# lturing/ORB_SLAM3_modified

Measured on AMD Instinct MI355X. Metric: ORB features/ms (+ frames/s), 640x480 8-level pyramid, 1000 features/frame, higher is better.
Workload: dtype u8

## Files before the change

### orb_slam3_modified_amd/csrc/orbx_kernels.hip

```cpp
#include <hip/hip_runtime.h>

#include "glibc_sincosf.h"
#include "gnu_sort.h"
#include "orbx_internal.h"

namespace orbx {

__constant__ __align__(16) int8_t c_pattern[1024] = {
#include "orb_pattern.inc"
};

__device__ __forceinline__ int fast_div(int n, uint32_t M) { return M ? (int)__umulhi((uint32_t)n, M) : n; }

__device__ __forceinline__ int mul_i24(int a, int b) {
  int r;
  asm("v_mul_i32_i24 %0, %1, %2" : "=v"(r) : "v"(a), "v"(b));
  return r;
}

__device__ __forceinline__ uint32_t mul_u24(uint32_t a, uint32_t b) {
  uint32_t r;
  asm("v_mul_u32_u24 %0, %1, %2" : "=v"(r) : "v"(a), "v"(b));
  return r;
}

__device__ __forceinline__ int xcd_logical_block(int n_items) {
  const int chunk = (int)(gridDim.x >> 3);
// ... 185 lines not shown
      *(uint32_t*)(B + r * bp + 4 * c) = v;
    }
  }
  __syncthreads();
#pragma unroll
  for (int k = 1; k <= K; k++) {
    const ChainLevel& L = a.lv[k - 1];
    const uint8_t* prev = smem + a.buf_off[k - 1];
    const int pp = a.buf_pitch[k - 1];
    const int nd = (X1[k] - X0[k] + 4) >> 2, nr = Y1[k] - Y0[k] + 1;
    uint8_t* outp = L.dst + (long long)frame * a.dst_frame_stride;
    const uint32_t m = nd > 1 ? (uint32_t)(((1ull << 32) + nd - 1) / nd) : 0u;
    for (int i = t; i < nd * nr; i += T) {
      const int r = fast_div(i, m), c = i - r * nd;
      const int y = Y0[k] + r, x4 = X0[k] + 4 * c;
      const uint32_t packed = chain_px4(prev, pp, X0[k - 1], Y0[k - 1], L.xt, L.yt[y], x4, L.w);
      if (x4 < ((L.w + 3) & ~3)) *(uint32_t*)(outp + (long long)y * L.pitch + x4) = packed;
      if (k < K) *(uint32_t*)(smem + a.buf_off[k] + r * a.buf_pitch[k] + 4 * c) = packed;
    }
    if (k < K) __syncthreads();
  }
}

__device__ __forceinline__ uint32_t umin3(uint32_t a, uint32_t b, uint32_t c) { return min(min(a, b), c); }
__device__ __forceinline__ uint32_t umax3(uint32_t a, uint32_t b, uint32_t c) { return max(max(a, b), c); }

__device__ __forceinline__ int fast_score16(int v, const uint32_t (&p)[16]) {
  uint32_t M3[16], m3[16];
#pragma unroll
  for (int k = 0; k < 16; k++) {
    M3[k] = umax3(p[k], p[(k + 1) & 15], p[(k + 2) & 15]);
    m3[k] = umin3(p[k], p[(k + 1) & 15], p[(k + 2) & 15]);
  }
  uint32_t M9[16], m9[16];
#pragma unroll
  for (int k = 0; k < 16; k++) {
    M9[k] = umax3(M3[k], M3[(k + 3) & 15], M3[(k + 6) & 15]);
    m9[k] = umin3(m3[k], m3[(k + 3) & 15], m3[(k + 6) & 15]);
  }
  uint32_t minmax = umin3(M9[0], M9[1], M9[2]), maxmin = umax3(m9[0], m9[1], m9[2]);
#pragma unroll
  for (int k = 3; k < 15; k += 2) {
    minmax = umin3(minmax, M9[k], M9[k + 1]);
    maxmin = umax3(maxmin, m9[k], m9[k + 1]);
  }
  minmax = min(minmax, M9[15]);
  maxmin = max(maxmin, m9[15]);
  return max(v - (int)minmax, (int)maxmin - v) - 1;
}

typedef unsigned short u16x2_t __attribute__((ext_vector_type(2)));
__device__ __forceinline__ u16x2_t as_u16x2(uint32_t x) { u16x2_t r; __builtin_memcpy(&r, &x, 4); return r; }
__device__ __forceinline__ uint32_t as_u32(u16x2_t x) { uint32_t r; __builtin_memcpy(&r, &x, 4); return r; }

__device__ __forceinline__ uint32_t fast_pretest_pk(uint32_t c, uint32_t p0, uint32_t p8, uint32_t p4, uint32_t p12, uint32_t p2,
                                                    uint32_t p10, uint32_t p6, uint32_t p14, uint32_t t_hi) {
  const u16x2_t a0 = as_u16x2(p0), a8 = as_u16x2(p8), a4 = as_u16x2(p4), a12 = as_u16x2(p12);
  const u16x2_t a2 = as_u16x2(p2), a10 = as_u16x2(p10), a6 = as_u16x2(p6), a14 = as_u16x2(p14);
  const u16x2_t maxmin = __builtin_elementwise_max(
      __builtin_elementwise_max(__builtin_elementwise_min(a0, a8), __builtin_elementwise_min(a4, a12)),
      __builtin_elementwise_max(__builtin_elementwise_min(a2, a10), __builtin_elementwise_min(a6, a14)));
  const u16x2_t minmax = __builtin_elementwise_min(
      __builtin_elementwise_min(__builtin_elementwise_max(a0, a8), __builtin_elementwise_max(a4, a12)),
      __builtin_elementwise_min(__builtin_elementwise_max(a2, a10), __builtin_elementwise_max(a6, a14)));
  const u16x2_t T = as_u16x2(t_hi);
  const u16x2_t lo = __builtin_elementwise_sub_sat(as_u16x2(c & 0xff00ff00u), T);
  const u16x2_t hi = __builtin_elementwise_add_sat(as_u16x2(c | 0x00ff00ffu), T);
  return as_u32(__builtin_elementwise_sub_sat(lo, maxmin)) | as_u32(__builtin_elementwise_sub_sat(minmax, hi));
}

__device__ __forceinline__ uint32_t fast_pretest_pk_lo(uint32_t c, uint32_t p0, uint32_t p8, uint32_t p4, uint32_t p12, uint32_t p2,
                                                       uint32_t p10, uint32_t p6, uint32_t p14, uint32_t t_lo) {
  const u16x2_t a0 = as_u16x2(p0), a8 = as_u16x2(p8), a4 = as_u16x2(p4), a12 = as_u16x2(p12);
  const u16x2_t a2 = as_u16x2(p2), a10 = as_u16x2(p10), a6 = as_u16x2(p6), a14 = as_u16x2(p14);
  const u16x2_t maxmin = __builtin_elementwise_max(
      __builtin_elementwise_max(__builtin_elementwise_min(a0, a8), __builtin_elementwise_min(a4, a12)),
// ... 124 lines not shown
        ps[j] = (dark | bright) & valid & (act != 0);
      }
      const unsigned long long b0 = __ballot(ps[0]), b1 = __ballot(ps[1]), b2 = __ballot(ps[2]), b3 = __ballot(ps[3]);
      const int n0 = __popcll(b0), n1_ = __popcll(b1), n2 = __popcll(b2), n3 = __popcll(b3);
      const int tot = n0 + n1_ + n2 + n3;
      if (tot) {
        int base = 0;
        if (lane == 0) base = atomicAdd(&s_cnt, tot);
        base = __builtin_amdgcn_readfirstlane(base);
        const int ent = c0 + (ry << 7);
        const int o0 = __builtin_amdgcn_mbcnt_hi((uint32_t)(b0 >> 32), __builtin_amdgcn_mbcnt_lo((uint32_t)b0, base));
        const int o1 = __builtin_amdgcn_mbcnt_hi((uint32_t)(b1 >> 32), __builtin_amdgcn_mbcnt_lo((uint32_t)b1, base + n0));
        const int o2 = __builtin_amdgcn_mbcnt_hi((uint32_t)(b2 >> 32), __builtin_amdgcn_mbcnt_lo((uint32_t)b2, base + n0 + n1_));
        const int o3 = __builtin_amdgcn_mbcnt_hi((uint32_t)(b3 >> 32), __builtin_amdgcn_mbcnt_lo((uint32_t)b3, base + n0 + n1_ + n2));
        if (ps[0]) list[o0] = (uint16_t)ent;
        if (ps[1]) list[o1] = (uint16_t)(ent + 1);
        if (ps[2]) list[o2] = (uint16_t)(ent + 2);
        if (ps[3]) list[o3] = (uint16_t)(ent + 3);
      }
    }
  }
  __syncthreads();
  n1 = s_cnt;
  for (int e = t; e < n1; e += T) {
    const int ent = list[e];
    const int x = ent & 127, y = ent >> 7;
    const uint8_t* c0 = tile + y * PITCH + (x + xo);
    const int v = c0[3 * PITCH + 3];
    uint32_t p[16];
    p[0] = c0[6 * PITCH + 3];  p[1] = c0[6 * PITCH + 4];  p[2] = c0[5 * PITCH + 5];  p[3] = c0[4 * PITCH + 6];
    p[4] = c0[3 * PITCH + 6];  p[5] = c0[2 * PITCH + 6];  p[6] = c0[1 * PITCH + 5];  p[7] = c0[4];
    p[8] = c0[3];              p[9] = c0[2];              p[10] = c0[1 * PITCH + 1]; p[11] = c0[2 * PITCH];
    p[12] = c0[3 * PITCH];     p[13] = c0[4 * PITCH];     p[14] = c0[5 * PITCH + 1]; p[15] = c0[6 * PITCH + 2];
    const int s = fast_score16(v, p);
    if (s >= TH && s > 0) sc[(y + 1) * PITCH + (x + 1)] = (uint8_t)s;
  }
  __syncthreads();
  int any_ini = 0;
  for (int e = t; e < n1; e += T) {
    const int ent = list[e];
    const int x = ent & 127, y = ent >> 7;
    const uint8_t* q = sc + y * PITCH + x;
    const int s = q[PITCH + 1];
    if (s > 0) {
      const int m = max(max(max((int)q[0], (int)q[1]), max((int)q[2], (int)q[PITCH])),
                        max(max((int)q[PITCH + 2], (int)q[2 * PITCH]), max((int)q[2 * PITCH + 1], (int)q[2 * PITCH + 2])));
      if (s > m) {
        list[e] = (uint16_t)(ent | 0x8000);
        any_ini |= twopass ? 1 : (int)(s >= ini_th);
      }
    }
  }
  const int use_ini = __syncthreads_or(any_ini);
  if (!twopass) { TH = use_ini ? ini_th : min_th; break; }
  if (use_ini || pass == 1 || ini_th == min_th) break;
  TH = min_th;
  if (t == 0) s_cnt = 0;
  __syncthreads();
// ... 1887 lines not shown
    if constexpr (LDSP) {
      const uint8_t* sp = s_patch[w * K + k];
      const int lctr = 18 * kDescSlicePitch + 18 + ((kx - 18) & 3);
      if (brief_fma) brief_taps<true, kDescSlicePitch>(sp, lctr, kDescSlicePitch, pat, a, b, t0, t1);
      else brief_taps<false, kDescSlicePitch>(sp, lctr, kDescSlicePitch, pat, a, b, t0, t1);
    } else {
      if (brief_fma) brief_taps<true, 0>(bplane, ctr, bp, pat, a, b, t0, t1);
      else brief_taps<false, 0>(bplane, ctr, bp, pat, a, b, t0, t1);
    }
    const unsigned long long b0 = __ballot(t0[0] < t1[0]), b1 = __ballot(t0[1] < t1[1]), b2 = __ballot(t0[2] < t1[2]), b3 = __ballot(t0[3] < t1[3]);
    uint32_t word = 0;
    asm("s_nop 4\n\tv_writelane_b32 %0, %1, 0\n\tv_writelane_b32 %0, %2, 1\n\tv_writelane_b32 %0, %3, 2\n\tv_writelane_b32 %0, %4, 3\n\t"
        "v_writelane_b32 %0, %5, 4\n\tv_writelane_b32 %0, %6, 5\n\tv_writelane_b32 %0, %7, 6\n\tv_writelane_b32 %0, %8, 7"
        : "+v"(word)
        : "s"((uint32_t)b0), "s"((uint32_t)(b0 >> 32)), "s"((uint32_t)b1), "s"((uint32_t)(b1 >> 32)), "s"((uint32_t)b2), "s"((uint32_t)(b2 >> 32)),
          "s"((uint32_t)b3), "s"((uint32_t)(b3 >> 32)));
    if (lane < 8) *(uint32_t*)(out_desc + ((long long)frame * g->out_cap + slot) * 32 + lane * 4) = word;
    if (mirror_desc && lane < 8) *(uint32_t*)(mirror_desc + ((long long)frame * g->out_cap + slot) * 32 + lane * 4) = word;
  }
}

constexpr int kFB_ROWS = 43, kFB_PITCH = 48, kFB_X0 = 24, kFB_Y0 = 21, kFB_HP_ROWS = 22, kFB_HP_COLS = 40, kFB_BPITCH = 40;
#include "fb_items.inc"

template <int K, int R>
__global__ __launch_bounds__(256) void k_describe_blur(const DeviceGeom* __restrict__ g, const uint8_t* __restrict__ imgs,
                                                       long long img_row_stride, long long img_frame_stride,
                                                       const uint8_t* __restrict__ pyr, long long pyr_frame_bytes,
                                                       const uint2* __restrict__ kp_list, const int32_t* __restrict__ counts,
                                                       orbx_keypoint* __restrict__ out_kps, uint8_t* __restrict__ out_desc,
                                                       BlurConsts bc, int groups_per_frame, int nitems, uint32_t m_gpf,
                                                       int atan_fma, int brief_fma) {
  const int lane = threadIdx.x & 63, w = __builtin_amdgcn_readfirstlane(threadIdx.x >> 6);
  const int L = xcd_logical_block(nitems);
  if (L < 0) return;
  const int frame = fast_div(L, m_gpf);
  const int total = counts[frame * 2];
  const int first = (L - frame * groups_per_frame) * R * 4 * K;
  if (first >= total) return;
  char4 pat[4];
#pragma unroll
  for (int q = 0; q < 4; q++) pat[q] = ((const char4*)c_pattern)[q * 64 + lane];
  int wu[4], wv[4];
  {
    const uint4 a = ((const uint4*)c_fb_w)[2 * lane], b = ((const uint4*)c_fb_w)[2 * lane + 1];
    wu[0] = (int)a.x; wu[1] = (int)a.y; wu[2] = (int)a.z; wu[3] = (int)a.w;
    wv[0] = (int)b.x; wv[1] = (int)b.y; wv[2] = (int)b.z; wv[3] = (int)b.w;
  }
  __shared__ __align__(16) uint8_t s_raw[4 * K][kFB_ROWS * kFB_PITCH + 16];
  __shared__ __align__(16) uint32_t s_hp[4][kFB_HP_ROWS * kFB_HP_COLS];
  int h_r0[3], h_r1[3], h_hp[3], v_hp[3], v_b[3];
  {
    uint32_t o[16];
#pragma unroll
    for (int i = 0; i < 4; i++) {
      const uint4 q = ((const uint4*)c_fb_off)[4 * lane + i];
      o[4 * i] = q.x; o[4 * i + 1] = q.y; o[4 * i + 2] = q.z; o[4 * i + 3] = q.w;
    }
#pragma unroll
    for (int t = 0; t < 3; t++) { h_r0[t] = (int)o[5 * t]; h_r1[t] = (int)o[5 * t + 1]; h_hp[t] = (int)o[5 * t + 2]; v_hp[t] = (int)o[5 * t + 3]; v_b[t] = (int)o[5 * t + 4]; }
  }
  __shared__ int s_mom[4 * K][2];
  __shared__ float s_trig[4 * K][3];
  uint32_t* hp = s_hp[w];
#pragma unroll 1
  for (int rnd = 0; rnd < R; rnd++) {
  const int gfirst = first + rnd * 4 * K;
  if (gfirst >= total) break;
  const int g0 = gfirst + w * K;
  const int nk = max(0, min(K, total - g0));
  uint2 rec = make_uint2(0u, 0u);
  if (lane < nk) rec = kp_list[(long long)frame * g->out_cap + g0 + lane];
  if (rnd) __syncthreads();
  int my_m01 = 0, my_m10 = 0;
  __builtin_amdgcn_sched_barrier(0);
  if (nk > 0) {
    bool fast[K];
#pragma unroll
    for (int k = 0; k < K; k++) {
      const int kk = min(k, nk - 1);
      const uint32_t p = __builtin_amdgcn_readlane(rec.x, kk);
      const int l = (int)(__builtin_amdgcn_readlane(rec.y, kk) & 0xffu);
      const DeviceLevel& lv = g->lv[l];
// ... 66 lines not shown
      const uint32_t dwv[4] = {a.x, a.y, b.x, b.y};
      int m10 = 0, m01 = 0;
#pragma unroll
      for (int i = 0; i < 4; i++) {
        const int px = (int)(dwv[i] ^ 0x80808080u);
        m10 = __builtin_amdgcn_sdot4(px, wu[i], m10, false);
        m01 = __builtin_amdgcn_sdot4(px, wv[i], m01, false);
      }
      m10 = __builtin_amdgcn_readlane(wave_sum_lane63(m10), 63);
      m01 = __builtin_amdgcn_readlane(wave_sum_lane63(m01), 63);
      if (lane == k) { my_m10 = m10; my_m01 = m01; }
    }
  }
  if (lane < nk) { s_mom[w * K + lane][0] = my_m01; s_mom[w * K + lane][1] = my_m10; }
  __syncthreads();
  if (w == 0 && lane < 4 * K) {
    const float ang = fast_atan2_deg((float)s_mom[lane][0], (float)s_mom[lane][1], atan_fma);
    const float factorPI = (float)(3.14159265358979323846 / 180.f);
    const float rad = __fmul_rn(ang, factorPI);
    s_trig[lane][0] = ang; s_trig[lane][1] = orbx_glibc::cosf_exact(rad); s_trig[lane][2] = orbx_glibc::sinf_exact(rad);
  }
  __syncthreads();
  float my_a = 0.f, my_b = 0.f;
  if (lane < nk) {
    my_a = s_trig[w * K + lane][1]; my_b = s_trig[w * K + lane][2];
    const int l = (int)(rec.y & 0xffu), slot = (int)(rec.y >> 8);
    const DeviceLevel& lv = g->lv[l];
    orbx_keypoint kp;
    float fx = (float)pt_x(rec.x), fy = (float)pt_y(rec.x);
    if (l != 0) { fx = __fmul_rn(fx, lv.scale); fy = __fmul_rn(fy, lv.scale); }
    kp.x = fx; kp.y = fy; kp.size = (float)lv.scaled_patch; kp.angle = s_trig[w * K + lane][0]; kp.response = (float)pt_s(rec.x);
    kp.octave = l; kp.class_id = -1;
    out_kps[(long long)frame * g->out_cap + slot] = kp;
  }
#pragma unroll 1
  for (int k = 0; k < nk; k++) {
    const int slot = (int)(__builtin_amdgcn_readlane(rec.y, k) >> 8);
    const float a = __uint_as_float(__builtin_amdgcn_readlane(__float_as_uint(my_a), k));
    const float b = __uint_as_float(__builtin_amdgcn_readlane(__float_as_uint(my_b), k));
    uint8_t* sp = s_raw[w * K + k];
#pragma unroll
    for (int t = 0; t < 3; t++) {
      uint32_t ha[4], hb[4];
      hrow4((const uint32_t*)(sp + h_r0[t]), bc, ha);
      hrow4((const uint32_t*)(sp + h_r1[t]), bc, hb);
      uint4 o;
      o.x = __builtin_amdgcn_perm(hb[0], ha[0], 0x05040100u); o.y = __builtin_amdgcn_perm(hb[1], ha[1], 0x05040100u);
      o.z = __builtin_amdgcn_perm(hb[2], ha[2], 0x05040100u); o.w = __builtin_amdgcn_perm(hb[3], ha[3], 0x05040100u);
      if (t < 2 || lane + 128 < kFB_NH) *(uint4*)((uint8_t*)hp + h_hp[t]) = o;
    }
    wave_lds_sync();
#pragma unroll
    for (int t = 0; t < 3; t++) {
      uint4 P[4];
#pragma unroll
      for (int q = 0; q < 4; q++) P[q] = *(const uint4*)((const uint8_t*)hp + v_hp[t] + q * (kFB_HP_COLS * 4));
      uint32_t e[4], o[4];
#pragma unroll
      for (int c = 0; c < 4; c++) {
        const uint32_t p0 = c == 0 ? P[0].x : c == 1 ? P[0].y : c == 2 ? P[0].z : P[0].w;
        const uint32_t p1 = c == 0 ? P[1].x : c == 1 ? P[1].y : c == 2 ? P[1].z : P[1].w;
        const uint32_t p2 = c == 0 ? P[2].x : c == 1 ? P[2].y : c == 2 ? P[2].z : P[2].w;
        const uint32_t p3 = c == 0 ? P[3].x : c == 1 ? P[3].y : c == 2 ? P[3].z : P[3].w;
        e[c] = udot2(p3, bc.we[3], udot2(p2, bc.we[2], udot2(p1, bc.we[1], udot2(p0, bc.we[0], bc.radd))));
        o[c] = udot2(p3, bc.wo[3], udot2(p2, bc.wo[2], udot2(p1, bc.wo[1], udot2(p0, bc.wo[0], bc.radd))));
      }
      const uint32_t pe = __builtin_amdgcn_perm(__builtin_amdgcn_perm(e[3], e[2], 0x0c0c0602u), __builtin_amdgcn_perm(e[1], e[0], 0x0c0c0602u), 0x05040100u);
      const uint32_t po = __builtin_amdgcn_perm(__builtin_amdgcn_perm(o[3], o[2], 0x0c0c0602u), __builtin_amdgcn_perm(o[1], o[0], 0x0c0c0602u), 0x05040100u);
      if (t < 2 || lane + 128 < kFB_NV) {
        *(uint32_t*)(sp + v_b[t]) = pe;
        *(uint32_t*)(sp + v_b[t] + kFB_BPITCH) = po;
      }
    }
    wave_lds_sync();
    int t0[4], t1[4];
    const int lctr = 18 * kFB_BPITCH + 20;
    char4 patk[4];
#pragma unroll
    for (int q = 0; q < 4; q++) {
      uint32_t pq;
      __builtin_memcpy(&pq, &pat[q], 4);
      asm volatile("" : "+v"(pq));
      __builtin_memcpy(&patk[q], &pq, 4);
    }
    if (brief_fma) brief_taps<true, kFB_BPITCH>(sp, lctr, kFB_BPITCH, patk, a, b, t0, t1);
    else brief_taps<false, kFB_BPITCH>(sp, lctr, kFB_BPITCH, patk, a, b, t0, t1);
    const unsigned long long b0 = __ballot(t0[0] < t1[0]), b1 = __ballot(t0[1] < t1[1]), b2 = __ballot(t0[2] < t1[2]), b3 = __ballot(t0[3] < t1[3]);
    uint32_t word = 0;
    asm("s_nop 4\n\tv_writelane_b32 %0, %1, 0\n\tv_writelane_b32 %0, %2, 1\n\tv_writelane_b32 %0, %3, 2\n\tv_writelane_b32 %0, %4, 3\n\t"
        "v_writelane_b32 %0, %5, 4\n\tv_writelane_b32 %0, %6, 5\n\tv_writelane_b32 %0, %7, 6\n\tv_writelane_b32 %0, %8, 7"
        : "+v"(word)
        : "s"((uint32_t)b0), "s"((uint32_t)(b0 >> 32)), "s"((uint32_t)b1), "s"((uint32_t)(b1 >> 32)), "s"((uint32_t)b2), "s"((uint32_t)(b2 >> 32)),
          "s"((uint32_t)b3), "s"((uint32_t)(b3 >> 32)));
    if (lane < 8) *(uint32_t*)(out_desc + ((long long)frame * g->out_cap + slot) * 32 + lane * 4) = word;
  }
// ... 109 lines not shown
```

Before: 331,700.

## Pack FAST scoring two-per-lane and bin vertical blur work by keypoint angle

FAST corner scoring now handles two candidates per thread. Pixel values are packed into f16x2 lanes and reinterpreted as f16 bit patterns, so packed min/max extrema can halve the scoring ALU work. The descriptor blur's vertical pass now reads per-lane offsets from precomputed angle-binned tables (16 orientation bins). Only the blurred pixels that the rotated BRIEF pattern can touch are computed, cutting three passes to two. The cost is a large constant table, per-keypoint bin lookup, and reliance on small-integer f16 bit patterns ordering correctly under min/max.

```diff
diff --git a/orb_slam3_modified_amd/csrc/fb_vbins.inc b/orb_slam3_modified_amd/csrc/fb_vbins.inc
--- /dev/null
+++ b/orb_slam3_modified_amd/csrc/fb_vbins.inc
@@ -0,0 +1,260 @@
+constexpr int kFB_VBINS = 16;
+constexpr int kFB_NV_BIN[kFB_VBINS] = {123, 120, 119, 118, 118, 119, 118, 116, 116, 120, 120, 121, 121, 120, 121, 124};
+__constant__ __align__(16) uint32_t c_fb_vbin_off[kFB_VBINS * 64 * 4] = {
+  48, 12, 1488, 732, 192, 88, 1504, 736, 208, 92, 1520, 740, 224, 96, 1536, 744,
+  336, 164, 1552, 748, 352, 168, 1568, 752, 368, 172, 1616, 804, 384, 176, 1632, 808,
+  400, 180, 1648, 812, 416, 184, 1664, 816, 432, 188, 1680, 820, 448, 192, 1696, 824,
+  496, 244, 1712, 828, 512, 248, 1728, 832, 528, 252, 1776, 884, 544, 256, 1792, 888,
+  560, 260, 1808, 892, 576, 264, 1824, 896, 592, 268, 1840, 900, 608, 272, 1856, 904,
+  656, 324, 1872, 908, 672, 328, 1888, 912, 688, 332, 1920, 960, 704, 336, 1936, 964,
+  720, 340, 1952, 968, 736, 344, 1968, 972, 752, 348, 1984, 976, 768, 352, 2000, 980,
+  784, 356, 2016, 984, 816, 404, 2032, 988, 832, 408, 2048, 992, 848, 412, 2096, 1044,
+  864, 416, 2112, 1048, 880, 420, 2128, 1052, 896, 424, 2144, 1056, 912, 428, 2160, 1060,
+  928, 432, 2176, 1064, 944, 436, 2192, 1068, 976, 484, 2208, 1072, 992, 488, 2256, 1124,
+  1008, 492, 2272, 1128, 1024, 496, 2288, 1132, 1040, 500, 2304, 1136, 1056, 504, 2320, 1140,
+  1072, 508, 2336, 1144, 1088, 512, 2352, 1148, 1136, 564, 2368, 1152, 1152, 568, 2416, 1204,
+  1168, 572, 2432, 1208, 1184, 576, 2448, 1212, 1200, 580, 2464, 1216, 1216, 584, 2480, 1220,
+  1232, 588, 2496, 1224, 1248, 592, 2512, 1228, 1296, 644, 2528, 1232, 1312, 648, 2640, 1300,
+  1328, 652, 2656, 1304, 1344, 656, 2672, 1308, 1360, 660, 2816, 1384, 1376, 664, 2816, 1384,
+  1392, 668, 2816, 1384, 1408, 672, 2816, 1384, 1456, 724, 2816, 1384, 1472, 728, 2816, 1384,
+  48, 12, 1488, 732, 64, 16, 1504, 736, 80, 20, 1520, 740, 208, 92, 1536, 744,
+  224, 96, 1552, 748, 240, 100, 1568, 752, 256, 104, 1584, 756, 352, 168, 1600, 800,
+  368, 172, 1616, 804, 384, 176, 1632, 808, 400, 180, 1648, 812, 416, 184, 1664, 816,
+  512, 248, 1680, 820, 528, 252, 1696, 824, 544, 256, 1712, 828, 560, 260, 1728, 832,
+  576, 264, 1760, 880, 592, 268, 1776, 884, 672, 328, 1792, 888, 688, 332, 1808, 892,
+  704, 336, 1824, 896, 720, 340, 1840, 900, 736, 344, 1856, 904, 752, 348, 1872, 908,
+  768, 352, 1888, 912, 832, 408, 1920, 960, 848, 412, 1936, 964, 864, 416, 1952, 968,
+  880, 420, 1968, 972, 896, 424, 1984, 976, 912, 428, 2000, 980, 928, 432, 2016, 984,
+  944, 436, 2032, 988, 976, 484, 2096, 1044, 992, 488, 2112, 1048, 1008, 492, 2128, 1052,
+  1024, 496, 2144, 1056, 1040, 500, 2160, 1060, 1056, 504, 2176, 1064, 1072, 508, 2192, 1068,
+  1088, 512, 2288, 1132, 1104, 516, 2304, 1136, 1136, 564, 2320, 1140, 1152, 568, 2336, 1144,
+  1168, 572, 2352, 1148, 1184, 576, 2448, 1212, 1200, 580, 2464, 1216, 1216, 584, 2480, 1220,
+  1232, 588, 2496, 1224, 1248, 592, 2512, 1228, 1264, 596, 2624, 1296, 1280, 640, 2640, 1300,
+  1296, 644, 2656, 1304, 1312, 648, 2784, 1376, 1328, 652, 2800, 1380, 1344, 656, 2816, 1384,
+  1360, 660, 2816, 1384, 1376, 664, 2816, 1384, 1392, 668, 2816, 1384, 1408, 672, 2816, 1384,
+  1424, 676, 2816, 1384, 1440, 720, 2816, 1384, 1456, 724, 2816, 1384, 1472, 728, 2816, 1384,
+  64, 16, 1504, 736, 80, 20, 1520, 740, 96, 24, 1536, 744, 224, 96, 1552, 748,
+  240, 100, 1568, 752, 256, 104, 1584, 756, 272, 108, 1616, 804, 368, 172, 1632, 808,
+  384, 176, 1648, 812, 400, 180, 1664, 816, 416, 184, 1680, 820, 432, 188, 1696, 824,
+  528, 252, 1712, 828, 544, 256, 1728, 832, 560, 260, 1744, 836, 576, 264, 1776, 884,
+  592, 268, 1792, 888, 656, 324, 1808, 892, 672, 328, 1824, 896, 688, 332, 1840, 900,
+  704, 336, 1856, 904, 720, 340, 1872, 908, 736, 344, 1888, 912, 752, 348, 1904, 916,
+  816, 404, 1952, 968, 832, 408, 1968, 972, 848, 412, 1984, 976, 864, 416, 2000, 980,
+  880, 420, 2016, 984, 896, 424, 2032, 988, 912, 428, 2048, 992, 960, 480, 2064, 996,
+  976, 484, 2112, 1048, 992, 488, 2128, 1052, 1008, 492, 2144, 1056, 1024, 496, 2160, 1060,
+  1040, 500, 2176, 1064, 1056, 504, 2192, 1068, 1072, 508, 2208, 1072, 1088, 512, 2272, 1128,
+  1120, 560, 2288, 1132, 1136, 564, 2304, 1136, 1152, 568, 2320, 1140, 1168, 572, 2336, 1144,
+  1184, 576, 2352, 1148, 1200, 580, 2448, 1212, 1216, 584, 2464, 1216, 1232, 588, 2480, 1220,
+  1248, 592, 2496, 1224, 1264, 596, 2608, 1292, 1280, 640, 2624, 1296, 1296, 644, 2640, 1300,
+  1312, 648, 2768, 1372, 1328, 652, 2784, 1376, 1344, 656, 2800, 1380, 1360, 660, 2800, 1380,
+  1376, 664, 2800, 1380, 1392, 668, 2800, 1380, 1408, 672, 2800, 1380, 1424, 676, 2800, 1380,
+  1440, 720, 2800, 1380, 1456, 724, 2800, 1380, 1472, 728, 2800, 1380, 1488, 732, 2800, 1380,
+  96, 24, 1504, 736, 112, 28, 1520, 740, 240, 100, 1536, 744, 256, 104, 1552, 748,
+  272, 108, 1568, 752, 336, 164, 1632, 808, 352, 168, 1648, 812, 368, 172, 1664, 816,
+  384, 176, 1680, 820, 400, 180, 1696, 824, 416, 184, 1712, 828, 432, 188, 1728, 832,
+  448, 192, 1792, 888, 496, 244, 1808, 892, 512, 248, 1824, 896, 528, 252, 1840, 900,
+  544, 256, 1856, 904, 560, 260, 1872, 908, 576, 264, 1888, 912, 592, 268, 1904, 916,
+  608, 272, 1952, 968, 656, 324, 1968, 972, 672, 328, 1984, 976, 688, 332, 2000, 980,
+  704, 336, 2016, 984, 720, 340, 2032, 988, 736, 344, 2048, 992, 752, 348, 2064, 996,
+  768, 352, 2112, 1048, 816, 404, 2128, 1052, 832, 408, 2144, 1056, 848, 412, 2160, 1060,
+  864, 416, 2176, 1064, 880, 420, 2192, 1068, 896, 424, 2208, 1072, 912, 428, 2224, 1076,
+  928, 432, 2272, 1128, 976, 484, 2288, 1132, 992, 488, 2304, 1136, 1008, 492, 2320, 1140,
+  1024, 496, 2336, 1144, 1040, 500, 2352, 1148, 1056, 504, 2368, 1152, 1072, 508, 2432, 1208,
+  1088, 512, 2448, 1212, 1136, 564, 2464, 1216, 1152, 568, 2480, 1220, 1168, 572, 2496, 1224,
+  1184, 576, 2512, 1228, 1200, 580, 2528, 1232, 1216, 584, 2592, 1288, 1232, 588, 2608, 1292,
+  1248, 592, 2624, 1296, 1296, 644, 2768, 1372, 1312, 648, 2768, 1372, 1328, 652, 2768, 1372,
+  1344, 656, 2768, 1372, 1360, 660, 2768, 1372, 1376, 664, 2768, 1372, 1392, 668, 2768, 1372,
+  1408, 672, 2768, 1372, 1456, 724, 2768, 1372, 1472, 728, 2768, 1372, 1488, 732, 2768, 1372,
+  48, 12, 1568, 752, 192, 88, 1616, 804, 208, 92, 1632, 808, 224, 96, 1648, 812,
+  352, 168, 1664, 816, 368, 172, 1680, 820, 384, 176, 1696, 824, 400, 180, 1712, 828,
+  416, 184, 1728, 832, 432, 188, 1776, 884, 448, 192, 1792, 888, 512, 248, 1808, 892,
+  528, 252, 1824, 896, 544, 256, 1840, 900, 560, 260, 1856, 904, 576, 264, 1872, 908,
+  592, 268, 1888, 912, 608, 272, 1936, 964, 672, 328, 1952, 968, 688, 332, 1968, 972,
+  704, 336, 1984, 976, 720, 340, 2000, 980, 736, 344, 2016, 984, 752, 348, 2032, 988,
+  768, 352, 2048, 992, 784, 356, 2096, 1044, 832, 408, 2112, 1048, 848, 412, 2128, 1052,
+  864, 416, 2144, 1056, 880, 420, 2160, 1060, 896, 424, 2176, 1064, 912, 428, 2192, 1068,
+  928, 432, 2208, 1072, 944, 436, 2256, 1124, 992, 488, 2272, 1128, 1008, 492, 2288, 1132,
+  1024, 496, 2304, 1136, 1040, 500, 2320, 1140, 1056, 504, 2336, 1144, 1072, 508, 2352, 1148,
+  1088, 512, 2368, 1152, 1104, 516, 2416, 1204, 1152, 568, 2432, 1208, 1168, 572, 2448, 1212,
+  1184, 576, 2464, 1216, 1200, 580, 2480, 1220, 1216, 584, 2496, 1224, 1232, 588, 2512, 1228,
+  1248, 592, 2528, 1232, 1296, 644, 2640, 1300, 1312, 648, 2656, 1304, 1328, 652, 2672, 1308,
+  1344, 656, 2816, 1384, 1360, 660, 2832, 1388, 1376, 664, 2832, 1388, 1392, 668, 2832, 1388,
+  1408, 672, 2832, 1388, 1456, 724, 2832, 1388, 1472, 728, 2832, 1388, 1488, 732, 2832, 1388,
+  1504, 736, 2832, 1388, 1520, 740, 2832, 1388, 1536, 744, 2832, 1388, 1552, 748, 2832, 1388,
+  48, 12, 1552, 748, 64, 16, 1568, 752, 80, 20, 1584, 756, 208, 92, 1600, 800,
+  224, 96, 1616, 804, 240, 100, 1632, 808, 256, 104, 1648, 812, 368, 172, 1664, 816,
+  384, 176, 1680, 820, 400, 180, 1696, 824, 416, 184, 1712, 828, 528, 252, 1728, 832,
+  544, 256, 1744, 836, 560, 260, 1760, 880, 576, 264, 1776, 884, 592, 268, 1792, 888,
+  672, 328, 1808, 892, 688, 332, 1824, 896, 704, 336, 1840, 900, 720, 340, 1856, 904,
+  736, 344, 1872, 908, 752, 348, 1888, 912, 768, 352, 1936, 964, 832, 408, 1952, 968,
+  848, 412, 1968, 972, 864, 416, 1984, 976, 880, 420, 2000, 980, 896, 424, 2016, 984,
+  912, 428, 2032, 988, 928, 432, 2048, 992, 944, 436, 2096, 1044, 992, 488, 2112, 1048,
+  1008, 492, 2128, 1052, 1024, 496, 2144, 1056, 1040, 500, 2160, 1060, 1056, 504, 2176, 1064,
+  1072, 508, 2192, 1068, 1088, 512, 2288, 1132, 1104, 516, 2304, 1136, 1136, 564, 2320, 1140,
+  1152, 568, 2336, 1144, 1168, 572, 2352, 1148, 1184, 576, 2448, 1212, 1200, 580, 2464, 1216,
+  1216, 584, 2480, 1220, 1232, 588, 2496, 1224, 1248, 592, 2512, 1228, 1264, 596, 2624, 1296,
+  1296, 644, 2640, 1300, 1312, 648, 2656, 1304, 1328, 652, 2672, 1308, 1344, 656, 2784, 1376,
+  1360, 660, 2800, 1380, 1376, 664, 2816, 1384, 1392, 668, 2960, 1460, 1408, 672, 2960, 1460,
+  1424, 676, 2960, 1460, 1440, 720, 2960, 1460, 1456, 724, 2960, 1460, 1472, 728, 2960, 1460,
+  1488, 732, 2960, 1460, 1504, 736, 2960, 1460, 1520, 740, 2960, 1460, 1536, 744, 2960, 1460,
+  80, 20, 1568, 752, 96, 24, 1584, 756, 224, 96, 1616, 804, 240, 100, 1632, 808,
+  256, 104, 1648, 812, 272, 108, 1664, 816, 384, 176, 1680, 820, 400, 180, 1696, 824,
+  416, 184, 1712, 828, 432, 188, 1728, 832, 528, 252, 1744, 836, 544, 256, 1776, 884,
+  560, 260, 1792, 888, 576, 264, 1808, 892, 592, 268, 1824, 896, 672, 328, 1840, 900,
+  688, 332, 1856, 904, 704, 336, 1872, 908, 720, 340, 1888, 912, 736, 344, 1904, 916,
+  752, 348, 1952, 968, 816, 404, 1968, 972, 832, 408, 1984, 976, 848, 412, 2000, 980,
+  864, 416, 2016, 984, 880, 420, 2032, 988, 896, 424, 2048, 992, 912, 428, 2064, 996,
+  928, 432, 2112, 1048, 976, 484, 2128, 1052, 992, 488, 2144, 1056, 1008, 492, 2160, 1060,
+  1024, 496, 2176, 1064, 1040, 500, 2192, 1068, 1056, 504, 2208, 1072, 1072, 508, 2272, 1128,
+  1088, 512, 2288, 1132, 1120, 560, 2304, 1136, 1136, 564, 2320, 1140, 1152, 568, 2336, 1144,
+  1168, 572, 2352, 1148, 1184, 576, 2448, 1212, 1200, 580, 2464, 1216, 1216, 584, 2480, 1220,
+  1232, 588, 2496, 1224, 1248, 592, 2608, 1292, 1280, 640, 2624, 1296, 1296, 644, 2640, 1300,
+  1312, 648, 2656, 1304, 1328, 652, 2768, 1372, 1344, 656, 2784, 1376, 1360, 660, 2800, 1380,
+  1376, 664, 2944, 1456, 1392, 668, 2960, 1460, 1408, 672, 2960, 1460, 1424, 676, 2960, 1460,
+  1440, 720, 2960, 1460, 1456, 724, 2960, 1460, 1472, 728, 2960, 1460, 1488, 732, 2960, 1460,
+  1504, 736, 2960, 1460, 1520, 740, 2960, 1460, 1536, 744, 2960, 1460, 1552, 748, 2960, 1460,
+  256, 104, 1648, 812, 272, 108, 1664, 816, 384, 176, 1680, 820, 400, 180, 1696, 824,
+  416, 184, 1712, 828, 432, 188, 1728, 832, 448, 192, 1792, 888, 496, 244, 1808, 892,
+  512, 248, 1824, 896, 528, 252, 1840, 900, 544, 256, 1856, 904, 560, 260, 1872, 908,
+  576, 264, 1888, 912, 592, 268, 1904, 916, 608, 272, 1952, 968, 656, 324, 1968, 972,
+  672, 328, 1984, 976, 688, 332, 2000, 980, 704, 336, 2016, 984, 720, 340, 2032, 988,
+  736, 344, 2048, 992, 752, 348, 2064, 996, 768, 352, 2112, 1048, 816, 404, 2128, 1052,
+  832, 408, 2144, 1056, 848, 412, 2160, 1060, 864, 416, 2176, 1064, 880, 420, 2192, 1068,
+  896, 424, 2208, 1072, 912, 428, 2224, 1076, 928, 432, 2272, 1128, 976, 484, 2288, 1132,
+  992, 488, 2304, 1136, 1008, 492, 2320, 1140, 1024, 496, 2336, 1144, 1040, 500, 2352, 1148,
+  1056, 504, 2368, 1152, 1072, 508, 2384, 1156, 1088, 512, 2432, 1208, 1136, 564, 2448, 1212,
+  1152, 568, 2464, 1216, 1168, 572, 2480, 1220, 1184, 576, 2496, 1224, 1200, 580, 2512, 1228,
+  1216, 584, 2528, 1232, 1232, 588, 2592, 1288, 1248, 592, 2608, 1292, 1296, 644, 2624, 1296,
+  1312, 648, 2640, 1300, 1328, 652, 2752, 1368, 1344, 656, 2768, 1372, 1360, 660, 2784, 1376,
+  1376, 664, 2784, 1376, 1392, 668, 2784, 1376, 1408, 672, 2784, 1376, 1456, 724, 2784, 1376,
+  1472, 728, 2784, 1376, 1488, 732, 2784, 1376, 1504, 736, 2784, 1376, 1520, 740, 2784, 1376,
+  1536, 744, 2784, 1376, 1552, 748, 2784, 1376, 1568, 752, 2784, 1376, 1632, 808, 2784, 1376,
+  192, 88, 1664, 816, 208, 92, 1680, 820, 224, 96, 1696, 824, 352, 168, 1712, 828,
+  368, 172, 1728, 832, 384, 176, 1776, 884, 400, 180, 1792, 888, 512, 248, 1808, 892,
+  528, 252, 1824, 896, 544, 256, 1840, 900, 560, 260, 1856, 904, 576, 264, 1872, 908,
+  592, 268, 1888, 912, 608, 272, 1936, 964, 672, 328, 1952, 968, 688, 332, 1968, 972,
+  704, 336, 1984, 976, 720, 340, 2000, 980, 736, 344, 2016, 984, 752, 348, 2032, 988,
+  768, 352, 2048, 992, 784, 356, 2096, 1044, 832, 408, 2112, 1048, 848, 412, 2128, 1052,
+  864, 416, 2144, 1056, 880, 420, 2160, 1060, 896, 424, 2176, 1064, 912, 428, 2192, 1068,
+  928, 432, 2208, 1072, 944, 436, 2256, 1124, 992, 488, 2272, 1128, 1008, 492, 2288, 1132,
+  1024, 496, 2304, 1136, 1040, 500, 2320, 1140, 1056, 504, 2336, 1144, 1072, 508, 2352, 1148,
+  1088, 512, 2368, 1152, 1104, 516, 2416, 1204, 1152, 568, 2432, 1208, 1168, 572, 2448, 1212,
+  1184, 576, 2464, 1216, 1200, 580, 2480, 1220, 1216, 584, 2496, 1224, 1232, 588, 2512, 1228,
+  1248, 592, 2528, 1232, 1296, 644, 2624, 1296, 1312, 648, 2640, 1300, 1328, 652, 2656, 1304,
+  1344, 656, 2672, 1308, 1360, 660, 2688, 1312, 1376, 664, 2816, 1384, 1392, 668, 2832, 1388,
+  1408, 672, 2832, 1388, 1456, 724, 2832, 1388, 1472, 728, 2832, 1388, 1488, 732, 2832, 1388,
+  1504, 736, 2832, 1388, 1520, 740, 2832, 1388, 1536, 744, 2832, 1388, 1552, 748, 2832, 1388,
+  1568, 752, 2832, 1388, 1616, 804, 2832, 1388, 1632, 808, 2832, 1388, 1648, 812, 2832, 1388,
+  64, 16, 1616, 804, 80, 20, 1632, 808, 208, 92, 1648, 812, 224, 96, 1664, 816,
+  240, 100, 1680, 820, 368, 172, 1696, 824, 384, 176, 1712, 828, 400, 180, 1728, 832,
+  416, 184, 1744, 836, 528, 252, 1760, 880, 544, 256, 1776, 884, 560, 260, 1792, 888,
+  576, 264, 1808, 892, 672, 328, 1824, 896, 688, 332, 1840, 900, 704, 336, 1856, 904,
+  720, 340, 1872, 908, 736, 344, 1888, 912, 752, 348, 1920, 960, 832, 408, 1936, 964,
+  848, 412, 1952, 968, 864, 416, 1968, 972, 880, 420, 1984, 976, 896, 424, 2000, 980,
+  912, 428, 2016, 984, 928, 432, 2032, 988, 944, 436, 2048, 992, 992, 488, 2096, 1044,
+  1008, 492, 2112, 1048, 1024, 496, 2128, 1052, 1040, 500, 2144, 1056, 1056, 504, 2160, 1060,
+  1072, 508, 2176, 1064, 1088, 512, 2192, 1068, 1104, 516, 2272, 1128, 1136, 564, 2288, 1132,
+  1152, 568, 2304, 1136, 1168, 572, 2320, 1140, 1184, 576, 2336, 1144, 1200, 580, 2352, 1148,
+  1216, 584, 2448, 1212, 1232, 588, 2464, 1216, 1248, 592, 2480, 1220, 1264, 596, 2496, 1224,
+  1296, 644, 2512, 1228, 1312, 648, 2608, 1292, 1328, 652, 2624, 1296, 1344, 656, 2640, 1300,
+  1360, 660, 2656, 1304, 1376, 664, 2672, 1308, 1392, 668, 2784, 1376, 1408, 672, 2800, 1380,
+  1424, 676, 2816, 1384, 1440, 720, 2944, 1456, 1456, 724, 2960, 1460, 1472, 728, 2976, 1464,
+  1488, 732, 2976, 1464, 1504, 736, 2976, 1464, 1520, 740, 2976, 1464, 1536, 744, 2976, 1464,
+  1552, 748, 2976, 1464, 1568, 752, 2976, 1464, 1584, 756, 2976, 1464, 1600, 800, 2976, 1464,
+  80, 20, 1584, 756, 96, 24, 1616, 804, 224, 96, 1632, 808, 240, 100, 1648, 812,
+  256, 104, 1664, 816, 384, 176, 1680, 820, 400, 180, 1696, 824, 416, 184, 1712, 828,
+  432, 188, 1728, 832, 528, 252, 1744, 836, 544, 256, 1776, 884, 560, 260, 1792, 888,
+  576, 264, 1808, 892, 592, 268, 1824, 896, 672, 328, 1840, 900, 688, 332, 1856, 904,
+  704, 336, 1872, 908, 720, 340, 1888, 912, 736, 344, 1904, 916, 752, 348, 1936, 964,
+  816, 404, 1952, 968, 832, 408, 1968, 972, 848, 412, 1984, 976, 864, 416, 2000, 980,
+  880, 420, 2016, 984, 896, 424, 2032, 988, 912, 428, 2048, 992, 960, 480, 2064, 996,
+  976, 484, 2112, 1048, 992, 488, 2128, 1052, 1008, 492, 2144, 1056, 1024, 496, 2160, 1060,
+  1040, 500, 2176, 1064, 1056, 504, 2192, 1068, 1072, 508, 2208, 1072, 1088, 512, 2272, 1128,
+  1120, 560, 2288, 1132, 1136, 564, 2304, 1136, 1152, 568, 2320, 1140, 1168, 572, 2336, 1144,
+  1184, 576, 2352, 1148, 1200, 580, 2432, 1208, 1216, 584, 2448, 1212, 1232, 588, 2464, 1216,
+  1248, 592, 2480, 1220, 1280, 640, 2496, 1224, 1296, 644, 2608, 1292, 1312, 648, 2624, 1296,
+  1328, 652, 2640, 1300, 1344, 656, 2656, 1304, 1360, 660, 2768, 1372, 1376, 664, 2784, 1376,
+  1392, 668, 2800, 1380, 1408, 672, 2928, 1452, 1424, 676, 2944, 1456, 1440, 720, 2960, 1460,
+  1456, 724, 2960, 1460, 1472, 728, 2960, 1460, 1488, 732, 2960, 1460, 1504, 736, 2960, 1460,
+  1520, 740, 2960, 1460, 1536, 744, 2960, 1460, 1552, 748, 2960, 1460, 1568, 752, 2960, 1460,
+  256, 104, 1616, 804, 272, 108, 1632, 808, 384, 176, 1648, 812, 400, 180, 1664, 816,
+  416, 184, 1680, 820, 432, 188, 1696, 824, 448, 192, 1712, 828, 496, 244, 1728, 832,
+  512, 248, 1776, 884, 528, 252, 1792, 888, 544, 256, 1808, 892, 560, 260, 1824, 896,
+  576, 264, 1840, 900, 592, 268, 1856, 904, 608, 272, 1872, 908, 656, 324, 1888, 912,
+  672, 328, 1936, 964, 688, 332, 1952, 968, 704, 336, 1968, 972, 720, 340, 1984, 976,
+  736, 344, 2000, 980, 752, 348, 2016, 984, 768, 352, 2032, 988, 816, 404, 2048, 992,
+  832, 408, 2064, 996, 848, 412, 2096, 1044, 864, 416, 2112, 1048, 880, 420, 2128, 1052,
+  896, 424, 2144, 1056, 912, 428, 2160, 1060, 928, 432, 2176, 1064, 960, 480, 2192, 1068,
+  976, 484, 2208, 1072, 992, 488, 2224, 1076, 1008, 492, 2256, 1124, 1024, 496, 2272, 1128,
+  1040, 500, 2288, 1132, 1056, 504, 2304, 1136, 1072, 508, 2320, 1140, 1088, 512, 2336, 1144,
+  1136, 564, 2352, 1148, 1152, 568, 2368, 1152, 1168, 572, 2416, 1204, 1184, 576, 2432, 1208,
+  1200, 580, 2448, 1212, 1216, 584, 2464, 1216, 1232, 588, 2480, 1220, 1248, 592, 2496, 1224,
+  1296, 644, 2512, 1228, 1312, 648, 2528, 1232, 1328, 652, 2576, 1284, 1344, 656, 2592, 1288,
+  1360, 660, 2608, 1292, 1376, 664, 2624, 1296, 1392, 668, 2640, 1300, 1408, 672, 2752, 1368,
+  1456, 724, 2768, 1372, 1472, 728, 2768, 1372, 1488, 732, 2768, 1372, 1504, 736, 2768, 1372,
+  1520, 740, 2768, 1372, 1536, 744, 2768, 1372, 1552, 748, 2768, 1372, 1568, 752, 2768, 1372,
+  192, 88, 1552, 748, 208, 92, 1568, 752, 224, 96, 1616, 804, 336, 164, 1632, 808,
+  352, 168, 1648, 812, 368, 172, 1664, 816, 384, 176, 1680, 820, 400, 180, 1696, 824,
+  496, 244, 1712, 828, 512, 248, 1728, 832, 528, 252, 1776, 884, 544, 256, 1792, 888,
+  560, 260, 1808, 892, 576, 264, 1824, 896, 592, 268, 1840, 900, 608, 272, 1856, 904,
+  656, 324, 1872, 908, 672, 328, 1888, 912, 688, 332, 1920, 960, 704, 336, 1936, 964,
+  720, 340, 1952, 968, 736, 344, 1968, 972, 752, 348, 1984, 976, 768, 352, 2000, 980,
+  816, 404, 2016, 984, 832, 408, 2032, 988, 848, 412, 2048, 992, 864, 416, 2080, 1040,
+  880, 420, 2096, 1044, 896, 424, 2112, 1048, 912, 428, 2128, 1052, 928, 432, 2144, 1056,
+  944, 436, 2160, 1060, 976, 484, 2176, 1064, 992, 488, 2192, 1068, 1008, 492, 2208, 1072,
+  1024, 496, 2256, 1124, 1040, 500, 2272, 1128, 1056, 504, 2288, 1132, 1072, 508, 2304, 1136,
+  1088, 512, 2320, 1140, 1104, 516, 2336, 1144, 1136, 564, 2352, 1148, 1152, 568, 2368, 1152,
+  1168, 572, 2416, 1204, 1184, 576, 2432, 1208, 1200, 580, 2448, 1212, 1216, 584, 2464, 1216,
+  1232, 588, 2480, 1220, 1248, 592, 2496, 1224, 1296, 644, 2512, 1228, 1312, 648, 2528, 1232,
+  1328, 652, 2640, 1300, 1344, 656, 2656, 1304, 1360, 660, 2672, 1308, 1376, 664, 2816, 1384,
+  1392, 668, 2832, 1388, 1408, 672, 2832, 1388, 1456, 724, 2832, 1388, 1472, 728, 2832, 1388,
+  1488, 732, 2832, 1388, 1504, 736, 2832, 1388, 1520, 740, 2832, 1388, 1536, 744, 2832, 1388,
+  48, 12, 1552, 748, 64, 16, 1568, 752, 208, 92, 1584, 756, 224, 96, 1600, 800,
+  240, 100, 1616, 804, 352, 168, 1632, 808, 368, 172, 1648, 812, 384, 176, 1664, 816,
+  400, 180, 1680, 820, 416, 184, 1696, 824, 512, 248, 1712, 828, 528, 252, 1728, 832,
+  544, 256, 1760, 880, 560, 260, 1776, 884, 576, 264, 1792, 888, 672, 328, 1808, 892,
+  688, 332, 1824, 896, 704, 336, 1840, 900, 720, 340, 1856, 904, 736, 344, 1872, 908,
+  752, 348, 1888, 912, 832, 408, 1920, 960, 848, 412, 1936, 964, 864, 416, 1952, 968,
+  880, 420, 1968, 972, 896, 424, 1984, 976, 912, 428, 2000, 980, 928, 432, 2016, 984,
+  944, 436, 2032, 988, 976, 484, 2096, 1044, 992, 488, 2112, 1048, 1008, 492, 2128, 1052,
+  1024, 496, 2144, 1056, 1040, 500, 2160, 1060, 1056, 504, 2176, 1064, 1072, 508, 2192, 1068,
+  1088, 512, 2272, 1128, 1104, 516, 2288, 1132, 1136, 564, 2304, 1136, 1152, 568, 2320, 1140,
+  1168, 572, 2336, 1144, 1184, 576, 2352, 1148, 1200, 580, 2448, 1212, 1216, 584, 2464, 1216,
+  1232, 588, 2480, 1220, 1248, 592, 2496, 1224, 1264, 596, 2512, 1228, 1280, 640, 2608, 1292,
+  1296, 644, 2624, 1296, 1312, 648, 2640, 1300, 1328, 652, 2656, 1304, 1344, 656, 2784, 1376,
+  1360, 660, 2800, 1380, 1376, 664, 2816, 1384, 1392, 668, 2944, 1456, 1408, 672, 2960, 1460,
+  1424, 676, 2960, 1460, 1440, 720, 2960, 1460, 1456, 724, 2960, 1460, 1472, 728, 2960, 1460,
+  1488, 732, 2960, 1460, 1504, 736, 2960, 1460, 1520, 740, 2960, 1460, 1536, 744, 2960, 1460,
+  64, 16, 1504, 736, 80, 20, 1520, 740, 96, 24, 1536, 744, 224, 96, 1552, 748,
+  240, 100, 1568, 752, 256, 104, 1584, 756, 368, 172, 1616, 804, 384, 176, 1632, 808,
+  400, 180, 1648, 812, 416, 184, 1664, 816, 432, 188, 1680, 820, 512, 248, 1696, 824,
+  528, 252, 1712, 828, 544, 256, 1728, 832, 560, 260, 1744, 836, 576, 264, 1776, 884,
+  592, 268, 1792, 888, 656, 324, 1808, 892, 672, 328, 1824, 896, 688, 332, 1840, 900,
+  704, 336, 1856, 904, 720, 340, 1872, 908, 736, 344, 1888, 912, 752, 348, 1904, 916,
+  800, 400, 1952, 968, 816, 404, 1968, 972, 832, 408, 1984, 976, 848, 412, 2000, 980,
+  864, 416, 2016, 984, 880, 420, 2032, 988, 896, 424, 2048, 992, 912, 428, 2064, 996,
+  960, 480, 2112, 1048, 976, 484, 2128, 1052, 992, 488, 2144, 1056, 1008, 492, 2160, 1060,
+  1024, 496, 2176, 1064, 1040, 500, 2192, 1068, 1056, 504, 2208, 1072, 1072, 508, 2272, 1128,
+  1088, 512, 2288, 1132, 1120, 560, 2304, 1136, 1136, 564, 2320, 1140, 1152, 568, 2336, 1144,
+  1168, 572, 2352, 1148, 1184, 576, 2432, 1208, 1200, 580, 2448, 1212, 1216, 584, 2464, 1216,
+  1232, 588, 2480, 1220, 1248, 592, 2496, 1224, 1280, 640, 2608, 1292, 1296, 644, 2624, 1296,
+  1312, 648, 2640, 1300, 1328, 652, 2768, 1372, 1344, 656, 2784, 1376, 1360, 660, 2800, 1380,
+  1376, 664, 2944, 1456, 1392, 668, 2944, 1456, 1408, 672, 2944, 1456, 1424, 676, 2944, 1456,
+  1440, 720, 2944, 1456, 1456, 724, 2944, 1456, 1472, 728, 2944, 1456, 1488, 732, 2944, 1456,
+  96, 24, 1488, 732, 240, 100, 1504, 736, 256, 104, 1520, 740, 272, 108, 1536, 744,
+  336, 164, 1552, 748, 352, 168, 1568, 752, 368, 172, 1616, 804, 384, 176, 1632, 808,
+  400, 180, 1648, 812, 416, 184, 1664, 816, 432, 188, 1680, 820, 448, 192, 1696, 824,
+  496, 244, 1712, 828, 512, 248, 1728, 832, 528, 252, 1776, 884, 544, 256, 1792, 888,
+  560, 260, 1808, 892, 576, 264, 1824, 896, 592, 268, 1840, 900, 608, 272, 1856, 904,
+  656, 324, 1872, 908, 672, 328, 1888, 912, 688, 332, 1936, 964, 704, 336, 1952, 968,
+  720, 340, 1968, 972, 736, 344, 1984, 976, 752, 348, 2000, 980, 768, 352, 2016, 984,
+  800, 400, 2032, 988, 816, 404, 2048, 992, 832, 408, 2064, 996, 848, 412, 2096, 1044,
+  864, 416, 2112, 1048, 880, 420, 2128, 1052, 896, 424, 2144, 1056, 912, 428, 2160, 1060,
+  928, 432, 2176, 1064, 960, 480, 2192, 1068, 976, 484, 2208, 1072, 992, 488, 2256, 1124,
+  1008, 492, 2272, 1128, 1024, 496, 2288, 1132, 1040, 500, 2304, 1136, 1056, 504, 2320, 1140,
+  1072, 508, 2336, 1144, 1088, 512, 2352, 1148, 1136, 564, 2368, 1152, 1152, 568, 2416, 1204,
+  1168, 572, 2432, 1208, 1184, 576, 2448, 1212, 1200, 580, 2464, 1216, 1216, 584, 2480, 1220,
+  1232, 588, 2496, 1224, 1248, 592, 2512, 1228, 1296, 644, 2528, 1232, 1312, 648, 2592, 1288,
+  1328, 652, 2608, 1292, 1344, 656, 2624, 1296, 1360, 660, 2752, 1368, 1376, 664, 2768, 1372,
+  1392, 668, 2768, 1372, 1408, 672, 2768, 1372, 1456, 724, 2768, 1372, 1472, 728, 2768, 1372,
+};
diff --git a/orb_slam3_modified_amd/csrc/orbx_kernels.hip b/orb_slam3_modified_amd/csrc/orbx_kernels.hip
--- a/orb_slam3_modified_amd/csrc/orbx_kernels.hip
+++ b/orb_slam3_modified_amd/csrc/orbx_kernels.hip
@@ -3,6 +3,7 @@
 #include "glibc_sincosf.h"
 #include "gnu_sort.h"
 #include "orbx_internal.h"
+#include "pk_f16_extrema.h"
 
 namespace orbx {
 
@@ -234,36 +235,39 @@
   }
 }
 
-__device__ __forceinline__ uint32_t umin3(uint32_t a, uint32_t b, uint32_t c) { return min(min(a, b), c); }
-__device__ __forceinline__ uint32_t umax3(uint32_t a, uint32_t b, uint32_t c) { return max(max(a, b), c); }
-
-__device__ __forceinline__ int fast_score16(int v, const uint32_t (&p)[16]) {
-  uint32_t M3[16], m3[16];
-#pragma unroll
-  for (int k = 0; k < 16; k++) {
-    M3[k] = umax3(p[k], p[(k + 1) & 15], p[(k + 2) & 15]);
-    m3[k] = umin3(p[k], p[(k + 1) & 15], p[(k + 2) & 15]);
-  }
-  uint32_t M9[16], m9[16];
-#pragma unroll
-  for (int k = 0; k < 16; k++) {
-    M9[k] = umax3(M3[k], M3[(k + 3) & 15], M3[(k + 6) & 15]);
-    m9[k] = umin3(m3[k], m3[(k + 3) & 15], m3[(k + 6) & 15]);
-  }
-  uint32_t minmax = umin3(M9[0], M9[1], M9[2]), maxmin = umax3(m9[0], m9[1], m9[2]);
-#pragma unroll
-  for (int k = 3; k < 15; k += 2) {
-    minmax = umin3(minmax, M9[k], M9[k + 1]);
-    maxmin = umax3(maxmin, m9[k], m9[k + 1]);
-  }
-  minmax = min(minmax, M9[15]);
-  maxmin = max(maxmin, m9[15]);
-  return max(v - (int)minmax, (int)maxmin - v) - 1;
-}
 
 typedef unsigned short u16x2_t __attribute__((ext_vector_type(2)));
 __device__ __forceinline__ u16x2_t as_u16x2(uint32_t x) { u16x2_t r; __builtin_memcpy(&r, &x, 4); return r; }
 __device__ __forceinline__ uint32_t as_u32(u16x2_t x) { uint32_t r; __builtin_memcpy(&r, &x, 4); return r; }
+
+__device__ __forceinline__ uint32_t fast_score16_pk(u16x2_t v, const h16x2_t (&p)[16]) {
+  h16x2_t M3[16], m3[16];
+#pragma unroll
+  for (int k = 0; k < 16; k++) {
+    M3[k] = hmax3(p[k], p[(k + 1) & 15], p[(k + 2) & 15]);
+    m3[k] = hmin3(p[k], p[(k + 1) & 15], p[(k + 2) & 15]);
+  }
+  h16x2_t M9[16], m9[16];
+#pragma unroll
+  for (int k = 0; k < 16; k++) {
+    M9[k] = hmax3(M3[k], M3[(k + 3) & 15], M3[(k + 6) & 15]);
+    m9[k] = hmin3(m3[k], m3[(k + 3) & 15], m3[(k + 6) & 15]);
+  }
+  h16x2_t minmax = hmin3(M9[0], M9[1], M9[2]), maxmin = hmax3(m9[0], m9[1], m9[2]);
+#pragma unroll
+  for (int k = 3; k < 15; k += 2) {
+    minmax = hmin3(minmax, M9[k], M9[k + 1]);
+    maxmin = hmax3(maxmin, m9[k], m9[k + 1]);
+  }
+  minmax = __builtin_elementwise_minimum(minmax, M9[15]);
+  maxmin = __builtin_elementwise_maximum(maxmin, m9[15]);
+  typedef short i16x2_t __attribute__((ext_vector_type(2)));
+  i16x2_t mm, Mm, V;
+  __builtin_memcpy(&mm, &minmax, 4); __builtin_memcpy(&Mm, &maxmin, 4); __builtin_memcpy(&V, &v, 4);
+  const i16x2_t s = __builtin_elementwise_max(V - mm, Mm - V) - (i16x2_t){1, 1};
+  uint32_t r; __builtin_memcpy(&r, &s, 4);
+  return r;
+}
 
 __device__ __forceinline__ uint32_t fast_pretest_pk(uint32_t c, uint32_t p0, uint32_t p8, uint32_t p4, uint32_t p12, uint32_t p2,
                                                     uint32_t p10, uint32_t p6, uint32_t p14, uint32_t t_hi) {
@@ -434,18 +438,22 @@
   }
   __syncthreads();
   n1 = s_cnt;
-  for (int e = t; e < n1; e += T) {
-    const int ent = list[e];
-    const int x = ent & 127, y = ent >> 7;
-    const uint8_t* c0 = tile + y * PITCH + (x + xo);
-    const int v = c0[3 * PITCH + 3];
-    uint32_t p[16];
-    p[0] = c0[6 * PITCH + 3];  p[1] = c0[6 * PITCH + 4];  p[2] = c0[5 * PITCH + 5];  p[3] = c0[4 * PITCH + 6];
-    p[4] = c0[3 * PITCH + 6];  p[5] = c0[2 * PITCH + 6];  p[6] = c0[1 * PITCH + 5];  p[7] = c0[4];
-    p[8] = c0[3];              p[9] = c0[2];              p[10] = c0[1 * PITCH + 1]; p[11] = c0[2 * PITCH];
-    p[12] = c0[3 * PITCH];     p[13] = c0[4 * PITCH];     p[14] = c0[5 * PITCH + 1]; p[15] = c0[6 * PITCH + 2];
-    const int s = fast_score16(v, p);
-    if (s >= TH && s > 0) sc[(y + 1) * PITCH + (x + 1)] = (uint8_t)s;
+  for (int e = 2 * t; e < n1; e += 2 * T) {
+    const int ent0 = list[e], has1 = e + 1 < n1, ent1 = has1 ? (int)list[e + 1] : ent0;
+    const int x0 = ent0 & 127, y0 = ent0 >> 7, x1 = ent1 & 127, y1 = ent1 >> 7;
+    const uint8_t* a = tile + y0 * PITCH + (x0 + xo);
+    const uint8_t* b = tile + y1 * PITCH + (x1 + xo);
+#define PK2(o) __builtin_bit_cast(h16x2_t, (u16x2_t){(unsigned short)a[o], (unsigned short)b[o]})
+    const u16x2_t v = {(unsigned short)a[3 * PITCH + 3], (unsigned short)b[3 * PITCH + 3]};
+    const h16x2_t p[16] = {PK2(6 * PITCH + 3), PK2(6 * PITCH + 4), PK2(5 * PITCH + 5), PK2(4 * PITCH + 6),
+                           PK2(3 * PITCH + 6), PK2(2 * PITCH + 6), PK2(1 * PITCH + 5), PK2(4),
+                           PK2(3),             PK2(2),             PK2(1 * PITCH + 1), PK2(2 * PITCH),
+                           PK2(3 * PITCH),     PK2(4 * PITCH),     PK2(5 * PITCH + 1), PK2(6 * PITCH + 2)};
+#undef PK2
+    const uint32_t s2 = fast_score16_pk(v, p);
+    const int s0 = (int)(short)(s2 & 0xffffu), s1 = (int)s2 >> 16;
+    if (s0 >= TH && s0 > 0) sc[(y0 + 1) * PITCH + (x0 + 1)] = (uint8_t)s0;
+    if (has1 && s1 >= TH && s1 > 0) sc[(y1 + 1) * PITCH + (x1 + 1)] = (uint8_t)s1;
   }
   __syncthreads();
   int any_ini = 0;
@@ -2379,6 +2387,7 @@
 
 constexpr int kFB_ROWS = 43, kFB_PITCH = 48, kFB_X0 = 24, kFB_Y0 = 21, kFB_HP_ROWS = 22, kFB_HP_COLS = 40, kFB_BPITCH = 40;
 #include "fb_items.inc"
+#include "fb_vbins.inc"
 
 template <int K, int R>
 __global__ __launch_bounds__(256) void k_describe_blur(const DeviceGeom* __restrict__ g, const uint8_t* __restrict__ imgs,
@@ -2406,7 +2415,7 @@
   }
   __shared__ __align__(16) uint8_t s_raw[4 * K][kFB_ROWS * kFB_PITCH + 16];
   __shared__ __align__(16) uint32_t s_hp[4][kFB_HP_ROWS * kFB_HP_COLS];
-  int h_r0[3], h_r1[3], h_hp[3], v_hp[3], v_b[3];
+  int h_r0[3], h_r1[3], h_hp[3];
   {
     uint32_t o[16];
 #pragma unroll
@@ -2415,7 +2424,7 @@
       o[4 * i] = q.x; o[4 * i + 1] = q.y; o[4 * i + 2] = q.z; o[4 * i + 3] = q.w;
     }
 #pragma unroll
-    for (int t = 0; t < 3; t++) { h_r0[t] = (int)o[5 * t]; h_r1[t] = (int)o[5 * t + 1]; h_hp[t] = (int)o[5 * t + 2]; v_hp[t] = (int)o[5 * t + 3]; v_b[t] = (int)o[5 * t + 4]; }
+    for (int t = 0; t < 3; t++) { h_r0[t] = (int)o[5 * t]; h_r1[t] = (int)o[5 * t + 1]; h_hp[t] = (int)o[5 * t + 2]; }
   }
   __shared__ int s_mom[4 * K][2];
   __shared__ float s_trig[4 * K][3];
@@ -2528,8 +2537,10 @@
   }
   __syncthreads();
   float my_a = 0.f, my_b = 0.f;
+  int my_bin = 0;
   if (lane < nk) {
     my_a = s_trig[w * K + lane][1]; my_b = s_trig[w * K + lane][2];
+    my_bin = min(kFB_VBINS - 1, max(0, (int)(s_trig[w * K + lane][0] * (kFB_VBINS / 360.f))));
     const int l = (int)(rec.y & 0xffu), slot = (int)(rec.y >> 8);
     const DeviceLevel& lv = g->lv[l];
     orbx_keypoint kp;
@@ -2545,6 +2556,7 @@
     const float a = __uint_as_float(__builtin_amdgcn_readlane(__float_as_uint(my_a), k));
     const float b = __uint_as_float(__builtin_amdgcn_readlane(__float_as_uint(my_b), k));
     uint8_t* sp = s_raw[w * K + k];
+    const uint4 vo = ((const uint4*)c_fb_vbin_off)[__builtin_amdgcn_readlane(my_bin, k) * 64 + lane];
 #pragma unroll
     for (int t = 0; t < 3; t++) {
       uint32_t ha[4], hb[4];
@@ -2557,10 +2569,11 @@
     }
     wave_lds_sync();
 #pragma unroll
-    for (int t = 0; t < 3; t++) {
+    for (int t = 0; t < 2; t++) {
+      const int v_hp = (int)(t ? vo.z : vo.x), v_b = (int)(t ? vo.w : vo.y);
       uint4 P[4];
 #pragma unroll
-      for (int q = 0; q < 4; q++) P[q] = *(const uint4*)((const uint8_t*)hp + v_hp[t] + q * (kFB_HP_COLS * 4));
+      for (int q = 0; q < 4; q++) P[q] = *(const uint4*)((const uint8_t*)hp + v_hp + q * (kFB_HP_COLS * 4));
       uint32_t e[4], o[4];
 #pragma unroll
       for (int c = 0; c < 4; c++) {
@@ -2573,10 +2586,8 @@
       }
       const uint32_t pe = __builtin_amdgcn_perm(__builtin_amdgcn_perm(e[3], e[2], 0x0c0c0602u), __builtin_amdgcn_perm(e[1], e[0], 0x0c0c0602u), 0x05040100u);
       const uint32_t po = __builtin_amdgcn_perm(__builtin_amdgcn_perm(o[3], o[2], 0x0c0c0602u), __builtin_amdgcn_perm(o[1], o[0], 0x0c0c0602u), 0x05040100u);
-      if (t < 2 || lane + 128 < kFB_NV) {
-        *(uint32_t*)(sp + v_b[t]) = pe;
-        *(uint32_t*)(sp + v_b[t] + kFB_BPITCH) = po;
-      }
+      *(uint32_t*)(sp + v_b) = pe;
+      *(uint32_t*)(sp + v_b + kFB_BPITCH) = po;
     }
     wave_lds_sync();
     int t0[4], t1[4];
diff --git a/orb_slam3_modified_amd/csrc/pk_f16_extrema.h b/orb_slam3_modified_amd/csrc/pk_f16_extrema.h
--- /dev/null
+++ b/orb_slam3_modified_amd/csrc/pk_f16_extrema.h
@@ -0,0 +1,15 @@
+#pragma once
+#include <hip/hip_runtime.h>
+
+namespace orbx {
+
+typedef _Float16 h16x2_t __attribute__((ext_vector_type(2)));
+
+__device__ __forceinline__ h16x2_t hmax3(h16x2_t a, h16x2_t b, h16x2_t c) {
+  return __builtin_elementwise_maximum(__builtin_elementwise_maximum(a, b), c);
+}
+__device__ __forceinline__ h16x2_t hmin3(h16x2_t a, h16x2_t b, h16x2_t c) {
+  return __builtin_elementwise_minimum(__builtin_elementwise_minimum(a, b), c);
+}
+
+}
```

Measured after the change: 336,600 (median of 6 runs). 1.5% higher.
